# Ewenwan/ORB_SLAM2_SSD_Semantic

Measured on AMD Instinct MI355X. Metric: ORB extract+match frames/sec on 640x480 TUM RGB-D; bit-exact kp/desc, higher is better.
Workload: dtype u8

## Files before the change

orb_slam2_ssd_semantic_amd/csrc/orbfe_api.hip:

```cpp
#include <stdarg.h>
#include <stdlib.h>

#include <algorithm>

#include "orbfe_extractor.h"

static thread_local char t_err[512] = "";

void orbfe_set_error(const char *fmt, ...)
{
    va_list ap;
    va_start(ap, fmt);
    vsnprintf(t_err, sizeof(t_err), fmt, ap);
    va_end(ap);
}

extern "C" const char *orbfe_last_error(void) { return t_err; }
extern "C" int32_t orbfe_version(void) { return ORBFE_VERSION; }

extern "C" const char *orbfe_strerror(orbfe_status s)
{
    switch (s) {
    case ORBFE_OK: return "ok";
    case ORBFE_ERR_ARG: return "invalid argument";
// ... 99 lines not shown
    *flags = 0;
    if (!h->d_misc.p) return ORBFE_OK;
    ORBFE_HIP(wait_last_call(h));
    ORBFE_HIP(hipMemcpy(flags, h->d_misc.p, sizeof(int32_t), hipMemcpyDeviceToHost));
    if (*flags) ORBFE_HIP(hipMemset(h->d_misc.p, 0, sizeof(int32_t)));
    return ORBFE_OK;
}

static orbfe_status create_impl(const orbfe_params *p, hipStream_t borrowed, hipStream_t borrowed_side, bool borrow, orbfe_handle **out);
extern "C" orbfe_status orbfe_create(const orbfe_params *p, orbfe_handle **out) { return create_impl(p, nullptr, nullptr, false, out); }
orbfe_status orbfe_internal_create_on_stream(const orbfe_params *p, void *st, void *side, orbfe_handle **out)
{
    return create_impl(p, (hipStream_t)st, (hipStream_t)side, true, out);
}

static orbfe_status create_impl(const orbfe_params *p, hipStream_t borrowed, hipStream_t borrowed_side, bool borrow, orbfe_handle **out)
{
    if (!p || !out) { orbfe_set_error("null argument"); return ORBFE_ERR_ARG; }
    *out = nullptr;
    OrbPlanIn pin;
    float sigma2[ORBFE_MAX_LEVELS] = {0}, inv_sigma2[ORBFE_MAX_LEVELS] = {0};
    const orbfe_status cs = orb_ctor_tables(p, &pin, sigma2, inv_sigma2);
    if (cs != ORBFE_OK) return cs;
    int dev = p->device;
    const orbfe_status rs = orb_resolve_device(&dev);
    if (rs != ORBFE_OK) return rs;

    orbfe_handle *h = new (std::nothrow) orbfe_handle();
    if (!h) return ORBFE_ERR_NOMEM;
    h->prm = *p;
    h->device = dev;
    DeviceGuard g(dev);
    h->pin = pin;
    memcpy(h->sigma2, sigma2, sizeof(sigma2));
    memcpy(h->inv_sigma2, inv_sigma2, sizeof(inv_sigma2));

    auto fail = [&](orbfe_status s) {
        orbfe_destroy(h);
        return s;
    };
    if (borrow) {
        h->stream = borrowed;
        h->own_stream = false;
        if (borrowed_side) {
            h->side = borrowed_side;
            h->own_side = false;
        }
    }
    for (int r = 0; r < ORBFE_PROF_RING; ++r)
        for (int i = 0; i < ORBFE_EV_N; ++i) h->ev[r][i] = nullptr;
    h->ev_ok = true;
    bool made = true;
    for (const OwnedStream &s : handle_streams(h))
        if (s.own) made = made && hipStreamCreateWithFlags(s.s, hipStreamNonBlocking) == hipSuccess;
    for (int r = 0; r < ORBFE_PROF_RING; ++r)
        for (int i = 0; i < ORBFE_EV_N; ++i) made = made && hipEventCreate(&h->ev[r][i]) == hipSuccess;
    for (hipEvent_t *e : handle_events(h)) made = made && hipEventCreateWithFlags(e, hipEventDisableTiming) == hipSuccess;
    if (!made || h->h_auto.ensure(64) != hipSuccess) {
        orbfe_set_error("stream / event creation failed: %s", hipGetErrorString(hipGetLastError()));
        return fail(ORBFE_ERR_HIP);
    }
#ifdef ORBFE_DEVELOPER
// ... 334 lines not shown
    auto finish = [&]() -> orbfe_status {
        if (ev) {
            ORBFE_HIP(hipEventRecord(ev[5], st));
            h->prof_calls++;
        }
        ORBFE_HIP(hipEventRecord(h->ev_last, st));
        h->last_stream = st;
        h->last_stream_valid = true;
        h->last_gray = d_gray;
        h->last_gray_fstride = (int64_t)frame_stride;
        h->last_gray_pitch = stride;
        h->last_nframes = nframes;
        return ORBFE_OK;
    };
    int ov = h->overlap >= 0 ? h->overlap : (nframes >= 128 ? 2 : 0);
#ifdef ORBFE_DEVELOPER
    if (h->pin.fuse_blur_pyr) {
        ORBFE_HIP(orbk_launch_blur_pyr(a, st));
        if (ev) {
            ORBFE_HIP(hipEventRecord(ev[1], st));
            ORBFE_HIP(hipEventRecord(ev[6], st));
            ORBFE_HIP(hipEventRecord(ev[7], st));
        }
        ORBFE_HIP(orbk_launch_fast(a, st));
        if (ev) ORBFE_HIP(hipEventRecord(ev[2], st));
        ORBFE_HIP(orbk_launch_octree(a, st));
        if (ev) {
            ORBFE_HIP(hipEventRecord(ev[3], st));
            ORBFE_HIP(hipEventRecord(ev[4], st));
        }
        ORBFE_HIP(orbk_launch_describe(a, st));
        return finish();
    }
    const bool ffp = h->fuse_fast_pyr == 1 || h->fuse_fast_pyr == 2;
    const bool fside = h->fuse_fast_pyr == 3;
    if (fside) {
        ORBFE_HIP(orbk_launch_fast_levels(a, 0, 0, 1, st));
        ORBFE_HIP(hipEventRecord(h->ev_fork2, st));
        ORBFE_HIP(hipStreamWaitEvent(h->side, h->ev_fork2, 0));
        ORBFE_HIP(orbk_launch_fast_levels(a, 0, 1, 0, h->side));
        ORBFE_HIP(hipEventRecord(h->ev_join2, h->side));
    }
    if ((ffp || fside) && ov == 1) ov = 2;
#else
    const bool ffp = false, fside = false;
    (void)fside;
#endif
    if (!ffp) ORBFE_HIP(orbk_launch_pyramid(a, st));
    if (ev) ORBFE_HIP(hipEventRecord(ev[1], st));
    auto fork_blur = [&]() -> hipError_t {
// ... 259 lines not shown
```

orb_slam2_ssd_semantic_amd/csrc/orbfe_kernels.h:

```cpp
#pragma once
#include "orbfe_common.h"

struct OrbOpts {
    int32_t pw_rows;
    int32_t pyr_fuse;
    int32_t qt[3];
};

struct OrbLaunch {
    OrbOpts opts;
    const OrbPlan *h_plan;
    const OrbPlan *d_plan;
    const OrbTab *d_tabs;
    const OrbLane *d_flanes;
    const OrbLane *d_flanes_c;
    const OrbLane *d_blanes;
    const OrbLaneR *d_blanesR;
    int32_t nframes;
    const uint8_t *d_gray;
    int64_t gray_fstride;
    int32_t gray_pitch;
    uint8_t *d_pyr;
    uint8_t *d_blur;
    int64_t pyr_fstride;
// ... 38 lines not shown
#endif

struct OrbPyrView {
    int32_t nlevels, device;
    const uint8_t *ptr[ORBFE_MAX_LEVELS];
    int32_t pitch[ORBFE_MAX_LEVELS], w[ORBFE_MAX_LEVELS], h[ORBFE_MAX_LEVELS];
    float scale[ORBFE_MAX_LEVELS], inv_scale[ORBFE_MAX_LEVELS];
    int64_t fstride[ORBFE_MAX_LEVELS];
    int32_t nframes;
};
hipError_t orbk_launch_pad_pyramid(const OrbPyrView &v, const uint32_t *off, uint8_t *d_out, hipStream_t st);
struct orbfe_handle;
int32_t orbfe_internal_pyramid_view(orbfe_handle *h, int frame, OrbPyrView *v);
int32_t orbfe_internal_order_after_last_call(orbfe_handle *h, void *stream);
orbfe_status orbfe_internal_create_on_stream(const orbfe_params *p, void *st, void *side, orbfe_handle **out);
```

orb_slam2_ssd_semantic_amd/csrc/orbfe_pipeline.hip:

```cpp
#include <new>
#include <vector>

#include "orbfe_common.h"
#include "orbfe_kernels.h"
#include "orbfe_matcher.h"

#ifndef ORBFE_PIPE_SIDE_STREAMS
#define ORBFE_PIPE_SIDE_STREAMS 1
#endif

struct orbfe_pipeline {
    orbfe_params prm;
    int device = 0;
    int P = 1;
    int F = 1;
    int cap = 0;
    std::vector<orbfe_handle *> ext;
    std::vector<orbfe_matcher *> mat;
    std::vector<hipStream_t> st;
    std::vector<hipStream_t> side;
    std::vector<hipEvent_t> ev_end;
    std::vector<hipEvent_t> ev_ext;
    std::vector<hipEvent_t> ev_match;
    std::vector<char> ev_match_valid;
    std::vector<char> ev_ext_valid;
    struct Slice { const char *k = nullptr, *d = nullptr, *n = nullptr; size_t kb = 0, db = 0, nb = 0; };
    std::vector<Slice> ev_slice;
    hipEvent_t ev_fork = nullptr;
    int32_t *d_seq = nullptr;
    int seq_len = 0;
    orbfe_keypoint *d_ckps[2] = {nullptr, nullptr};
    uint8_t *d_cdesc[2] = {nullptr, nullptr};
    int32_t *d_cn[2] = {nullptr, nullptr};
    hipEvent_t ev_carry[2] = {nullptr, nullptr};
    hipEvent_t ev_m0[2] = {nullptr, nullptr};
// ... 1 lines not shown
    bool carry_written[2] = {false, false};
    int carry_cur = 0;
    bool have_carry = false;
    const void *carry_src[3] = {nullptr, nullptr, nullptr};
    size_t carry_src_bytes[3] = {0, 0, 0};
    bool joined = true;
    int rot = 0;
    int host_pipes = 1;
    static const int NSETS = 3;
    uint8_t *d_in[NSETS] = {nullptr, nullptr, nullptr};
    orbfe_keypoint *d_okps[NSETS] = {nullptr, nullptr, nullptr};
    uint8_t *d_odesc[NSETS] = {nullptr, nullptr, nullptr};
    int32_t *d_on[NSETS] = {nullptr, nullptr, nullptr}, *d_om[NSETS] = {nullptr, nullptr, nullptr}, *d_onm[NSETS] = {nullptr, nullptr, nullptr};
    size_t in_bytes = 0;
    int out_frames = 0;
    hipStream_t s_in = nullptr, s_out = nullptr;
    hipEvent_t ev_out[NSETS] = {nullptr, nullptr, nullptr};
};

static orbfe_status ensure_events(orbfe_pipeline *pl, int nsub)
{
    while ((int)pl->ev_ext.size() < nsub) {
        hipEvent_t a = nullptr, b = nullptr;
        ORBFE_HIP(hipEventCreateWithFlags(&a, hipEventDisableTiming));
        pl->ev_ext.push_back(a);
        ORBFE_HIP(hipEventCreateWithFlags(&b, hipEventDisableTiming));
        pl->ev_match.push_back(b);
        pl->ev_match_valid.push_back(0);
        pl->ev_ext_valid.push_back(0);
        pl->ev_slice.push_back(orbfe_pipeline::Slice());
    }
    return ORBFE_OK;
}

static orbfe_status ensure_seq(orbfe_pipeline *pl, int nframes)
{
    if (nframes + 1 <= pl->seq_len) return ORBFE_OK;
    for (hipStream_t s : pl->st) ORBFE_HIP(hipStreamSynchronize(s));
    if (pl->d_seq) ORBFE_HIP(hipFree(pl->d_seq));
    pl->d_seq = nullptr;
    pl->seq_len = 0;
    const int len = std::max(nframes + 1, 4096);
    std::vector<int32_t> h((size_t)len);
    for (int i = 0; i < len; ++i) h[(size_t)i] = i - 1;
    ORBFE_HIP(hipMalloc((void **)&pl->d_seq, (size_t)len * sizeof(int32_t)));
    ORBFE_HIP(hipMemcpy(pl->d_seq, h.data(), (size_t)len * sizeof(int32_t), hipMemcpyHostToDevice));
    pl->seq_len = len;
    return ORBFE_OK;
}

extern "C" void orbfe_pipeline_destroy(orbfe_pipeline *pl)
{
    if (!pl) return;
    DeviceGuard g(pl->device);
    for (hipStream_t s : pl->st)
        if (s) (void)hipStreamSynchronize(s);
    for (orbfe_handle *h : pl->ext) orbfe_destroy(h);
    for (orbfe_matcher *m : pl->mat) orbfe_matcher_destroy(m);
    for (hipEvent_t e : pl->ev_end)
        if (e) (void)hipEventDestroy(e);
    for (hipEvent_t e : pl->ev_ext)
        if (e) (void)hipEventDestroy(e);
    for (hipEvent_t e : pl->ev_match)
        if (e) (void)hipEventDestroy(e);
    if (pl->ev_fork) (void)hipEventDestroy(pl->ev_fork);
    for (int k = 0; k < 2; ++k) {
        if (pl->ev_carry[k]) (void)hipEventDestroy(pl->ev_carry[k]);
        if (pl->ev_m0[k]) (void)hipEventDestroy(pl->ev_m0[k]);
        if (pl->d_ckps[k]) (void)hipFree(pl->d_ckps[k]);
        if (pl->d_cdesc[k]) (void)hipFree(pl->d_cdesc[k]);
        if (pl->d_cn[k]) (void)hipFree(pl->d_cn[k]);
    }
    if (pl->d_seq) (void)hipFree(pl->d_seq);
    if (pl->s_in) (void)hipStreamSynchronize(pl->s_in);
    if (pl->s_out) (void)hipStreamSynchronize(pl->s_out);
    for (int k = 0; k < orbfe_pipeline::NSETS; ++k) {
        void *bufs[] = {pl->d_in[k], pl->d_okps[k], pl->d_odesc[k], pl->d_on[k], pl->d_om[k], pl->d_onm[k]};
        for (void *b : bufs)
            if (b) (void)hipFree(b);
        if (pl->ev_out[k]) (void)hipEventDestroy(pl->ev_out[k]);
    }
    if (pl->s_in) (void)hipStreamDestroy(pl->s_in);
    if (pl->s_out) (void)hipStreamDestroy(pl->s_out);
    for (hipStream_t s : pl->st)
        if (s) (void)hipStreamDestroy(s);
    for (hipStream_t s : pl->side)
        if (s) (void)hipStreamDestroy(s);
    delete pl;
}

extern "C" orbfe_status orbfe_pipeline_create(const orbfe_params *p, int32_t npipes, orbfe_pipeline **out)
{
    if (!p || !out || npipes < 1 || npipes > 64) {
        orbfe_set_error("bad argument to orbfe_pipeline_create (1..64 pipes)");
        return ORBFE_ERR_ARG;
    }
    *out = nullptr;
    orbfe_pipeline *pl = new (std::nothrow) orbfe_pipeline();
    if (!pl) return ORBFE_ERR_NOMEM;
    pl->prm = *p;
    pl->P = npipes;
    pl->F = p->max_batch;
    auto fail = [&](orbfe_status s) {
        orbfe_pipeline_destroy(pl);
        return s;
    };
    {
        int dev = p->device;
        const orbfe_status rs = orb_resolve_device(&dev);
        if (rs != ORBFE_OK) return fail(rs);
        pl->device = dev;
        pl->prm.device = dev;
    }
    DeviceGuard g(pl->device);
    for (int i = 0; i < npipes; ++i) {
        hipStream_t st = nullptr;
        hipEvent_t e = nullptr;
        if (hipStreamCreateWithFlags(&st, hipStreamNonBlocking) != hipSuccess) { orbfe_set_error("pipeline stream creation failed"); return fail(ORBFE_ERR_HIP); }
        pl->st.push_back(st);
        if (hipEventCreateWithFlags(&e, hipEventDisableTiming) != hipSuccess) { orbfe_set_error("pipeline event creation failed"); return fail(ORBFE_ERR_HIP); }
        pl->ev_end.push_back(e);
    }
    for (int i = 0; i < std::min(npipes, ORBFE_PIPE_SIDE_STREAMS); ++i) {
        hipStream_t st = nullptr;
        if (hipStreamCreateWithFlags(&st, hipStreamNonBlocking) != hipSuccess) { orbfe_set_error("pipeline stream creation failed"); return fail(ORBFE_ERR_HIP); }
        pl->side.push_back(st);
    }
    for (int i = 0; i < npipes; ++i) {
        orbfe_handle *h = nullptr;
        orbfe_status s = orbfe_internal_create_on_stream(&pl->prm, (void *)pl->st[(size_t)i], (void *)pl->side[(size_t)i % pl->side.size()], &h);
        if (s != ORBFE_OK) return fail(s);
        pl->ext.push_back(h);
        orbfe_matcher *m = nullptr;
        s = orbfe_internal_matcher_create_on_stream(pl->device, (void *)pl->st[(size_t)i], &m);
        if (s != ORBFE_OK) return fail(s);
        pl->mat.push_back(m);
    }
    {
        int32_t feat[ORBFE_MAX_LEVELS];
        int worst = 0;
        if (orbfe_get_features_per_level(pl->ext[0], feat) == ORBFE_OK)
            for (int l = 0; l < pl->prm.nlevels; ++l) worst += std::max(feat[l] + 2, 4 * ORBFE_MAX_ROOTS);
        pl->cap = std::max(orbfe_keypoint_capacity(pl->ext[0]), (worst + 63) & ~63);
    }
    if (hipEventCreateWithFlags(&pl->ev_fork, hipEventDisableTiming) != hipSuccess) { orbfe_set_error("pipeline event creation failed"); return fail(ORBFE_ERR_HIP); }
    for (int k = 0; k < 2; ++k) {
        if (hipEventCreateWithFlags(&pl->ev_carry[k], hipEventDisableTiming) != hipSuccess ||
            hipEventCreateWithFlags(&pl->ev_m0[k], hipEventDisableTiming) != hipSuccess ||
            hipMalloc((void **)&pl->d_ckps[k], (size_t)pl->cap * sizeof(orbfe_keypoint)) != hipSuccess ||
            hipMalloc((void **)&pl->d_cdesc[k], (size_t)pl->cap * 32) != hipSuccess ||
            hipMalloc((void **)&pl->d_cn[k], 64) != hipSuccess) {
            orbfe_set_error("pipeline carry buffers: %s", hipGetErrorString(hipGetLastError()));
            return fail(ORBFE_ERR_NOMEM);
        }
        (void)hipMemset(pl->d_cn[k], 0, 64);
    }
    orbfe_status s = ensure_seq(pl, 4095);
    if (s != ORBFE_OK) return fail(s);
    *out = pl;
    return ORBFE_OK;
}

extern "C" int32_t orbfe_pipeline_pipes(const orbfe_pipeline *pl) { return pl ? pl->P : 0; }
extern "C" int32_t orbfe_pipeline_capacity(const orbfe_pipeline *pl) { return pl ? pl->cap : 0; }
extern "C" int32_t orbfe_pipeline_sub_batch(const orbfe_pipeline *pl) { return pl ? pl->F : 0; }
extern "C" orbfe_handle *orbfe_pipeline_extractor(orbfe_pipeline *pl, int32_t pipe)
{
    return (pl && pipe >= 0 && pipe < pl->P) ? pl->ext[(size_t)pipe] : nullptr;
}
extern "C" orbfe_matcher *orbfe_pipeline_matcher(orbfe_pipeline *pl, int32_t pipe)
{
    return (pl && pipe >= 0 && pipe < pl->P) ? pl->mat[(size_t)pipe] : nullptr;
}

extern "C" orbfe_status orbfe_pipeline_set_host_pipes(orbfe_pipeline *pl, int32_t n)
{
    if (!pl || n < 1) return ORBFE_ERR_ARG;
    pl->host_pipes = std::min(n, pl->P);
    return ORBFE_OK;
}

extern "C" orbfe_status orbfe_pipeline_reset_sequence(orbfe_pipeline *pl)
{
    if (!pl) return ORBFE_ERR_ARG;
    pl->have_carry = false;
    return ORBFE_OK;
}

extern "C" orbfe_status orbfe_pipeline_join(orbfe_pipeline *pl, void *stream)
{
    if (!pl) return ORBFE_ERR_ARG;
    DeviceGuard g(pl->device);
    for (int p = 0; p < pl->P; ++p) ORBFE_HIP(hipStreamWaitEvent((hipStream_t)stream, pl->ev_end[(size_t)p], 0));
    pl->joined = true;
    return ORBFE_OK;
}

extern "C" orbfe_status orbfe_pipeline_synchronize(orbfe_pipeline *pl)
{
    if (!pl) return ORBFE_ERR_ARG;
    DeviceGuard g(pl->device);
    for (hipStream_t s : pl->st) ORBFE_HIP(hipStreamSynchronize(s));
    return ORBFE_OK;
}

extern "C" orbfe_status orbfe_pipeline_get_overflow(orbfe_pipeline *pl, int32_t *flags)
{
    if (!pl || !flags) return ORBFE_ERR_ARG;
    *flags = 0;
    for (orbfe_handle *h : pl->ext) {
        int32_t f = 0;
        const orbfe_status s = orbfe_get_overflow(h, &f);
        if (s != ORBFE_OK) return s;
        *flags |= f;
    }
    return ORBFE_OK;
}

extern "C" orbfe_status orbfe_pipeline_extract_match_device(orbfe_pipeline *pl, const uint8_t *d_gray, int32_t nframes, int32_t w,
                                                            int32_t ht, int32_t stride, size_t frame_stride, orbfe_keypoint *d_kps,
                                                            uint8_t *d_desc, int32_t cap, int32_t *d_n_out, int32_t *d_match,
                                                            int32_t *d_nmatches, float nnratio, int32_t th, int32_t check_ori,
                                                            int32_t flags, void *stream)
{
    if (!pl || !d_gray || !d_kps || !d_desc || !d_n_out || nframes < 1 || cap < 1 || (d_match && !d_nmatches)) {
        orbfe_set_error("bad argument to orbfe_pipeline_extract_match_device");
        return ORBFE_ERR_ARG;
    }
    DeviceGuard g(pl->device);
    const int F = pl->F, P = pl->P;
    const int nsub = (nframes + F - 1) / F;
    orbfe_status s = ensure_events(pl, nsub + 1);
    if (s != ORBFE_OK) return s;
    s = ensure_seq(pl, nframes);
    if (s != ORBFE_OK) return s;
    hipStream_t cs = (hipStream_t)stream;
    const bool match = d_match != nullptr;
    const bool cont = (flags & ORBFE_PIPE_CONTINUE) != 0 && pl->have_carry && match;
    const int rd = pl->carry_cur, wr = pl->carry_cur ^ 1;

    ORBFE_HIP(hipEventRecord(pl->ev_fork, cs));
    for (int p = 0; p < P; ++p) ORBFE_HIP(hipStreamWaitEvent(pl->st[(size_t)p], pl->ev_fork, 0));
    auto bail = [&](orbfe_status e) {
        for (hipStream_t x : pl->st) (void)hipStreamSynchronize(x);
        pl->have_carry = false;
        pl->m0_valid[0] = pl->m0_valid[1] = false;
        pl->joined = true;
        return e;
    };
    auto overlaps = [](const void *a, size_t na, const void *b, size_t nb) {
        const char *pa = (const char *)a, *pb = (const char *)b;
        return a && b && pa < pb + nb && pb < pa + na;
    };

    for (int j = 0; j < nsub; ++j) {
        const int p = (pl->rot + j) % P;
        hipStream_t st = pl->st[(size_t)p];
        const int lo = j * F, nf = std::min(F, nframes - lo);
        {
            const char *ok = (const char *)(d_kps + (size_t)lo * cap), *od = (const char *)(d_desc + (size_t)lo * cap * 32), *on = (const char *)(d_n_out + lo);
            const size_t okb = (size_t)nf * cap * sizeof(orbfe_keypoint), odb = (size_t)nf * cap * 32, onb = (size_t)nf * sizeof(int32_t);
            auto wait_index = [&](size_t i) -> hipError_t {
                hipError_t e = hipSuccess;
                if (pl->ev_ext_valid[i]) e = hipStreamWaitEvent(st, pl->ev_ext[i], 0);
                if (e == hipSuccess && pl->ev_match_valid[i]) e = hipStreamWaitEvent(st, pl->ev_match[i], 0);
                if (e == hipSuccess && i + 1 < pl->ev_match_valid.size() && pl->ev_match_valid[i + 1]) e = hipStreamWaitEvent(st, pl->ev_match[i + 1], 0);
                return e;
            };
            ORBFE_HIP(wait_index((size_t)j));
            for (size_t i = 0; i < pl->ev_slice.size(); ++i) {
                const orbfe_pipeline::Slice &si = pl->ev_slice[i];
                if ((int)i != j && si.k && (overlaps(si.k, si.kb, ok, okb) || overlaps(si.d, si.db, od, odb) || overlaps(si.n, si.nb, on, onb)))
// ... 33 lines not shown
                                                 pl->d_seq + 1, pl->d_seq + 1, 1, nnratio, th, check_ori, d_match, d_nmatches, (void *)st);
                if (s != ORBFE_OK) return bail(s);
                ORBFE_HIP(hipEventRecord(pl->ev_m0[rd], st));
                pl->m0_valid[rd] = true;
            } else {
                ORBFE_HIP(hipMemsetAsync(d_match, 0xFF, (size_t)cap * sizeof(int32_t), st));
                ORBFE_HIP(hipMemsetAsync(d_nmatches, 0, sizeof(int32_t), st));
            }
        }
        ORBFE_HIP(hipEventRecord(pl->ev_match[(size_t)j], st));
        pl->ev_match_valid[(size_t)j] = 1;
    }

    {
        const int jl = nsub - 1;
        hipStream_t st = pl->st[(size_t)((pl->rot + jl) % P)];
        const size_t last = (size_t)nframes - 1;
        if (pl->m0_valid[wr]) {
            ORBFE_HIP(hipStreamWaitEvent(st, pl->ev_m0[wr], 0));
            pl->m0_valid[wr] = false;
        }
        if (pl->carry_written[wr]) ORBFE_HIP(hipStreamWaitEvent(st, pl->ev_carry[wr], 0));
        ORBFE_HIP(hipMemcpyAsync(pl->d_ckps[wr], d_kps + last * cap, (size_t)std::min(cap, pl->cap) * sizeof(orbfe_keypoint),
                                 hipMemcpyDeviceToDevice, st));
        ORBFE_HIP(hipMemcpyAsync(pl->d_cdesc[wr], d_desc + last * cap * 32, (size_t)std::min(cap, pl->cap) * 32, hipMemcpyDeviceToDevice, st));
        ORBFE_HIP(hipMemcpyAsync(pl->d_cn[wr], d_n_out + last, sizeof(int32_t), hipMemcpyDeviceToDevice, st));
        ORBFE_HIP(hipEventRecord(pl->ev_carry[wr], st));
        pl->carry_written[wr] = true;
        pl->carry_cur = wr;
        pl->have_carry = true;
        pl->carry_src[0] = d_kps + last * cap;
        pl->carry_src_bytes[0] = (size_t)std::min(cap, pl->cap) * sizeof(orbfe_keypoint);
        pl->carry_src[1] = d_desc + last * cap * 32;
        pl->carry_src_bytes[1] = (size_t)std::min(cap, pl->cap) * 32;
        pl->carry_src[2] = d_n_out + last;
        pl->carry_src_bytes[2] = sizeof(int32_t);
    }
    for (int p = 0; p < P; ++p) ORBFE_HIP(hipEventRecord(pl->ev_end[(size_t)p], pl->st[(size_t)p]));
    pl->joined = false;
    pl->rot = (pl->rot + nsub) % P;
    if (!(flags & ORBFE_PIPE_NO_JOIN)) return orbfe_pipeline_join(pl, stream);
    return ORBFE_OK;
}

static orbfe_status ensure_host_sets(orbfe_pipeline *pl, int w, int ht)
{
    const size_t need = (size_t)pl->F * w * ht;
    if (need <= pl->in_bytes && pl->out_frames == pl->F) return ORBFE_OK;
    if (!pl->s_in) ORBFE_HIP(hipStreamCreateWithFlags(&pl->s_in, hipStreamNonBlocking));
    if (!pl->s_out) ORBFE_HIP(hipStreamCreateWithFlags(&pl->s_out, hipStreamNonBlocking));
    ORBFE_HIP(hipStreamSynchronize(pl->s_in));
    ORBFE_HIP(hipStreamSynchronize(pl->s_out));
    for (hipStream_t st : pl->st) ORBFE_HIP(hipStreamSynchronize(st));
    const size_t F = (size_t)pl->F, cap = (size_t)pl->cap;
    for (int k = 0; k < orbfe_pipeline::NSETS; ++k) {
        if (pl->d_in[k]) ORBFE_HIP(hipFree(pl->d_in[k]));
        pl->d_in[k] = nullptr;
        ORBFE_HIP(hipMalloc((void **)&pl->d_in[k], need + 64));
        if (!pl->ev_out[k]) ORBFE_HIP(hipEventCreateWithFlags(&pl->ev_out[k], hipEventDisableTiming));
        if (!pl->d_okps[k]) {
            ORBFE_HIP(hipMalloc((void **)&pl->d_okps[k], F * cap * sizeof(orbfe_keypoint)));
            ORBFE_HIP(hipMalloc((void **)&pl->d_odesc[k], F * cap * 32));
            ORBFE_HIP(hipMalloc((void **)&pl->d_on[k], F * sizeof(int32_t)));
            ORBFE_HIP(hipMalloc((void **)&pl->d_om[k], F * cap * sizeof(int32_t)));
            ORBFE_HIP(hipMalloc((void **)&pl->d_onm[k], F * sizeof(int32_t)));
        }
    }
    pl->in_bytes = need;
// ... 3 lines not shown

extern "C" orbfe_status orbfe_pipeline_extract_match(orbfe_pipeline *pl, const uint8_t *const *grays, int32_t nframes, int32_t w, int32_t ht,
                                                     int32_t stride, orbfe_keypoint *kps, uint8_t *desc, int32_t cap, int32_t *n_out,
                                                     int32_t *match, int32_t *nmatches, float nnratio, int32_t th, int32_t check_ori,
                                                     int32_t flags)
{
    if (!pl || !grays || !kps || !desc || !n_out || nframes < 1 || w < 1 || ht < 1 || stride < w || (match && !nmatches)) {
        orbfe_set_error("bad argument to orbfe_pipeline_extract_match");
        return ORBFE_ERR_ARG;
    }
    if (cap < pl->cap) {
        orbfe_set_error("orbfe_pipeline_extract_match: cap %d below orbfe_pipeline_capacity() = %d", cap, pl->cap);
        return ORBFE_ERR_CAP;
    }
    DeviceGuard g(pl->device);
    orbfe_status s = ensure_host_sets(pl, w, ht);
    if (s != ORBFE_OK) return s;
    const int F = pl->F, pc = pl->cap;
    const size_t fbytes = (size_t)w * ht;
    const int nchunks = (nframes + F - 1) / F;
    struct Drain {
        orbfe_pipeline *pl;
        ~Drain()
        {
            if (pl->s_in) (void)hipStreamSynchronize(pl->s_in);
            for (hipStream_t st : pl->st) (void)hipStreamSynchronize(st);
            if (pl->s_out) (void)hipStreamSynchronize(pl->s_out);
        }
    } drain{pl};
    for (int c = 0; c < nchunks; ++c) {
        const int k = c % orbfe_pipeline::NSETS, lo = c * F, nf = std::min(F, nframes - lo);
        if (c >= orbfe_pipeline::NSETS) ORBFE_HIP(hipStreamWaitEvent(pl->s_in, pl->ev_out[k], 0));
        bool contiguous = stride == w;
        for (int f = 1; f < nf && contiguous; ++f) contiguous = grays[lo + f] == grays[lo + f - 1] + fbytes;
        if (contiguous) {
            ORBFE_HIP(hipMemcpyAsync(pl->d_in[k], grays[lo], fbytes * nf, hipMemcpyHostToDevice, pl->s_in));
        } else {
            for (int f = 0; f < nf; ++f)
                ORBFE_HIP(hipMemcpy2DAsync(pl->d_in[k] + fbytes * f, (size_t)w, grays[lo + f], (size_t)stride, (size_t)w, (size_t)ht,
                                           hipMemcpyHostToDevice, pl->s_in));
        }
        const int fl = ((c > 0 || (flags & ORBFE_PIPE_CONTINUE)) ? ORBFE_PIPE_CONTINUE : 0) | ORBFE_PIPE_NO_JOIN;
        pl->rot = c % std::max(1, std::min(pl->host_pipes, pl->P));
        s = orbfe_pipeline_extract_match_device(pl, pl->d_in[k], nf, w, ht, w, fbytes, pl->d_okps[k], pl->d_odesc[k], pc, pl->d_on[k],
                                                match ? pl->d_om[k] : nullptr, match ? pl->d_onm[k] : nullptr, nnratio, th, check_ori, fl,
                                                (void *)pl->s_in);
        if (s != ORBFE_OK) return s;
        s = orbfe_pipeline_join(pl, (void *)pl->s_out);
        if (s != ORBFE_OK) return s;
        ORBFE_HIP(hipMemcpyAsync(n_out + lo, pl->d_on[k], (size_t)nf * sizeof(int32_t), hipMemcpyDeviceToHost, pl->s_out));
        auto rows_out = [&](void *dst, const void *src, size_t elem) -> hipError_t {
            if (cap == pc) return hipMemcpyAsync(dst, src, (size_t)nf * pc * elem, hipMemcpyDeviceToHost, pl->s_out);
            return hipMemcpy2DAsync(dst, (size_t)cap * elem, src, (size_t)pc * elem, (size_t)pc * elem, (size_t)nf, hipMemcpyDeviceToHost, pl->s_out);
        };
        ORBFE_HIP(rows_out(kps + (size_t)lo * cap, pl->d_okps[k], sizeof(orbfe_keypoint)));
        ORBFE_HIP(rows_out(desc + (size_t)lo * cap * 32, pl->d_odesc[k], 32));
        if (match) {
            ORBFE_HIP(rows_out(match + (size_t)lo * cap, pl->d_om[k], sizeof(int32_t)));
            ORBFE_HIP(hipMemcpyAsync(nmatches + lo, pl->d_onm[k], (size_t)nf * sizeof(int32_t), hipMemcpyDeviceToHost, pl->s_out));
        }
        ORBFE_HIP(hipEventRecord(pl->ev_out[k], pl->s_out));
    }
    ORBFE_HIP(hipStreamSynchronize(pl->s_out));
    int32_t ovf = 0;
    s = orbfe_pipeline_get_overflow(pl, &ovf);
    if (s != ORBFE_OK) return s;
    if (ovf) {
        orbfe_set_error("device-side capacity overflow %d in orbfe_pipeline_extract_match", ovf);
        return ORBFE_ERR_CAP;
    }
    return ORBFE_OK;
}
```

orb_slam2_ssd_semantic_amd/pipeline.py:

```python
import ctypes as C

from . import _ffi
from ._ffi import Handle, OrbfeParams, check
from .extractor import ORBextractor
from .matcher import ORBmatcher


class FramePipeline(Handle):
    _HANDLE, _DESTROY = "_p", "orbfe_pipeline_destroy"
    CONTINUE, NO_JOIN = _ffi.PIPE_CONTINUE, _ffi.PIPE_NO_JOIN

    def __init__(self, nfeatures=1000, scaleFactor=1.2, nlevels=8, iniThFAST=20, minThFAST=7, *, max_width=640, max_height=480,
                 sub_batch=1024, npipes=3, device=-1, blur_rounding=0, nnratio=0.9, th=100, check_ori=True):
        self._L = _ffi.lib()
        self._p = C.c_void_p()
        prm = OrbfeParams(nfeatures, scaleFactor, nlevels, iniThFAST, minThFAST, max_width, max_height, sub_batch, device,
                          blur_rounding)
        check(self._L.orbfe_pipeline_create(C.byref(prm), npipes, C.byref(self._p)), "orbfe_pipeline_create")
        self.npipes, self.sub_batch, self.blur_rounding = npipes, sub_batch, blur_rounding
        self.cap = int(self._L.orbfe_pipeline_capacity(self._p))
        self.nnratio, self.th, self.check_ori = float(nnratio), int(th), bool(check_ori)
        kw = dict(max_width=max_width, max_height=max_height, max_batch=sub_batch, device=device, blur_rounding=blur_rounding)
        self.extractors = [ORBextractor(nfeatures, scaleFactor, nlevels, iniThFAST, minThFAST,
                                        _borrow=self._L.orbfe_pipeline_extractor(self._p, i), **kw) for i in range(npipes)]
        self.matchers = [ORBmatcher(nnratio, check_ori, _borrow=self._L.orbfe_pipeline_matcher(self._p, i)) for i in range(npipes)]

    def close(self):
        if getattr(self, "_p", None):
            for o in self.extractors + self.matchers:
                o.close()
        super().close()

    @property
# ... 5 lines not shown

    def extract_match_device(self, d_gray, nframes, w, h, stride, frame_stride, d_kps, d_desc, cap, d_n, d_match=None, d_nmatches=None,
                             flags=0, stream=None):
        check(self._L.orbfe_pipeline_extract_match_device(self._p, d_gray, nframes, w, h, stride, frame_stride, d_kps, d_desc, cap, d_n,
                                                          d_match, d_nmatches, self.nnratio, self.th, int(self.check_ori), flags,
                                                          stream), "orbfe_pipeline_extract_match_device")

    def extract_match(self, frame_ptrs, nframes, w, h, stride, kps_ptr, desc_ptr, cap, n_ptr, match_ptr=None, nmatches_ptr=None, flags=0):
        check(self._L.orbfe_pipeline_extract_match(self._p, frame_ptrs, nframes, w, h, stride, kps_ptr, desc_ptr, cap, n_ptr, match_ptr,
                                                   nmatches_ptr, self.nnratio, self.th, int(self.check_ori), flags),
              "orbfe_pipeline_extract_match")

    def set_host_pipes(self, n):
        check(self._L.orbfe_pipeline_set_host_pipes(self._p, int(n)), "orbfe_pipeline_set_host_pipes")

    def join(self, stream=None):
        check(self._L.orbfe_pipeline_join(self._p, stream), "orbfe_pipeline_join")

    def synchronize(self):
        check(self._L.orbfe_pipeline_synchronize(self._p), "orbfe_pipeline_synchronize")

    def reset_sequence(self):
        check(self._L.orbfe_pipeline_reset_sequence(self._p), "orbfe_pipeline_reset_sequence")

    def overflow(self):
        f = C.c_int32(0)
        check(self._L.orbfe_pipeline_get_overflow(self._p, C.byref(f)), "orbfe_pipeline_get_overflow")
        return f.value

    def set_fast_mode(self, mode, collect_stats=False):
# ... 7 lines not shown
```

Baseline: 307,100.

## Plan pipeline streams to fit the hardware queue count and reuse spare streams

```diff
diff --git a/orb_slam2_ssd_semantic_amd/csrc/orbfe_api.hip b/orb_slam2_ssd_semantic_amd/csrc/orbfe_api.hip
--- a/orb_slam2_ssd_semantic_amd/csrc/orbfe_api.hip
+++ b/orb_slam2_ssd_semantic_amd/csrc/orbfe_api.hip
@@ -137,6 +137,13 @@
     return create_impl(p, (hipStream_t)st, (hipStream_t)side, true, out);
 }
 
+orbfe_status orbfe_internal_set_side_stream(orbfe_handle *h, void *side)
+{
+    if (!h || h->own_side) return ORBFE_ERR_ARG;
+    h->side = (hipStream_t)side;
+    return ORBFE_OK;
+}
+
 static orbfe_status create_impl(const orbfe_params *p, hipStream_t borrowed, hipStream_t borrowed_side, bool borrow, orbfe_handle **out)
 {
     if (!p || !out) { orbfe_set_error("null argument"); return ORBFE_ERR_ARG; }
@@ -165,10 +172,8 @@
     if (borrow) {
         h->stream = borrowed;
         h->own_stream = false;
-        if (borrowed_side) {
-            h->side = borrowed_side;
-            h->own_side = false;
-        }
+        h->side = borrowed_side;
+        h->own_side = false;
     }
     for (int r = 0; r < ORBFE_PROF_RING; ++r)
         for (int i = 0; i < ORBFE_EV_N; ++i) h->ev[r][i] = nullptr;
@@ -533,6 +538,7 @@
         return ORBFE_OK;
     };
     int ov = h->overlap >= 0 ? h->overlap : (nframes >= 128 ? 2 : 0);
+    if (!h->side) ov = 0;
 #ifdef ORBFE_DEVELOPER
     if (h->pin.fuse_blur_pyr) {
         ORBFE_HIP(orbk_launch_blur_pyr(a, st));
@@ -552,7 +558,7 @@
         return finish();
     }
     const bool ffp = h->fuse_fast_pyr == 1 || h->fuse_fast_pyr == 2;
-    const bool fside = h->fuse_fast_pyr == 3;
+    const bool fside = h->fuse_fast_pyr == 3 && h->side;
     if (fside) {
         ORBFE_HIP(orbk_launch_fast_levels(a, 0, 0, 1, st));
         ORBFE_HIP(hipEventRecord(h->ev_fork2, st));
diff --git a/orb_slam2_ssd_semantic_amd/csrc/orbfe_kernels.h b/orb_slam2_ssd_semantic_amd/csrc/orbfe_kernels.h
--- a/orb_slam2_ssd_semantic_amd/csrc/orbfe_kernels.h
+++ b/orb_slam2_ssd_semantic_amd/csrc/orbfe_kernels.h
@@ -76,3 +76,4 @@
 int32_t orbfe_internal_pyramid_view(orbfe_handle *h, int frame, OrbPyrView *v);
 int32_t orbfe_internal_order_after_last_call(orbfe_handle *h, void *stream);
 orbfe_status orbfe_internal_create_on_stream(const orbfe_params *p, void *st, void *side, orbfe_handle **out);
+orbfe_status orbfe_internal_set_side_stream(orbfe_handle *h, void *side);
diff --git a/orb_slam2_ssd_semantic_amd/csrc/orbfe_pipe_plan.h b/orb_slam2_ssd_semantic_amd/csrc/orbfe_pipe_plan.h
--- /dev/null
+++ b/orb_slam2_ssd_semantic_amd/csrc/orbfe_pipe_plan.h
@@ -0,0 +1,58 @@
+#pragma once
+
+#include <errno.h>
+#include <stdint.h>
+#include <stdlib.h>
+
+#define ORBFE_PIPE_MAX_PIPES 64
+#define ORBFE_PIPE_DEFAULT_QUEUES 4
+#define ORBFE_PIPE_MAX_QUEUES 32
+#define ORBFE_PIPE_COPY_STREAMS 2
+
+struct OrbPipePlan {
+    int32_t P, Q, copies;
+    int32_t S;
+    int32_t P_eff;
+    int32_t side;
+    int32_t first, side_index , nstreams;
+    int32_t stream_of_pipe[ORBFE_PIPE_MAX_PIPES];
+};
+
+static inline int32_t orb_pipe_parse_queues(const char *text)
+{
+    if (!text || !*text) return ORBFE_PIPE_DEFAULT_QUEUES;
+    char *end = nullptr;
+    errno = 0;
+    const long long v = strtoll(text, &end, 10);
+    if (end == text) return ORBFE_PIPE_DEFAULT_QUEUES;
+    while (*end == ' ' || *end == '\t' || *end == '\n' || *end == '\r') ++end;
+    if (*end) return ORBFE_PIPE_DEFAULT_QUEUES;
+    if (errno == ERANGE) return v > 0 ? ORBFE_PIPE_MAX_QUEUES : ORBFE_PIPE_DEFAULT_QUEUES;
+    if (v < 1) return ORBFE_PIPE_DEFAULT_QUEUES;
+    return v > ORBFE_PIPE_MAX_QUEUES ? ORBFE_PIPE_MAX_QUEUES : (int32_t)v;
+}
+
+static inline int32_t orb_pipe_env_queues()
+{
+    static const int32_t q = orb_pipe_parse_queues(getenv("GPU_MAX_HW_QUEUES"));
+    return q;
+}
+
+static inline bool orb_pipe_plan(int32_t P, int32_t Q, bool copies, OrbPipePlan *out)
+{
+    if (!out || P < 1 || P > ORBFE_PIPE_MAX_PIPES) return false;
+    OrbPipePlan pl;
+    pl.P = P;
+    pl.Q = Q < 1 ? 1 : (Q > ORBFE_PIPE_MAX_QUEUES ? ORBFE_PIPE_MAX_QUEUES : Q);
+    pl.copies = copies ? 1 : 0;
+    pl.first = copies ? ORBFE_PIPE_COPY_STREAMS : 0;
+    const int32_t left = pl.Q - pl.first < 1 ? 1 : pl.Q - pl.first;
+    pl.side = left >= 2 ? 1 : 0;
+    pl.S = left >= P + 1 ? P : (pl.side ? left - 1 : 1);
+    pl.P_eff = P < pl.S ? P : pl.S;
+    pl.side_index = pl.side ? pl.first + pl.S : -1;
+    pl.nstreams = pl.first + pl.S + pl.side;
+    for (int32_t i = 0; i < ORBFE_PIPE_MAX_PIPES; ++i) pl.stream_of_pipe[i] = i < P ? i % pl.S : -1;
+    *out = pl;
+    return true;
+}
diff --git a/orb_slam2_ssd_semantic_amd/csrc/orbfe_pipeline.hip b/orb_slam2_ssd_semantic_amd/csrc/orbfe_pipeline.hip
--- a/orb_slam2_ssd_semantic_amd/csrc/orbfe_pipeline.hip
+++ b/orb_slam2_ssd_semantic_amd/csrc/orbfe_pipeline.hip
@@ -1,24 +1,43 @@
+#include <mutex>
 #include <new>
+#include <utility>
 #include <vector>
 
 #include "orbfe_common.h"
 #include "orbfe_kernels.h"
 #include "orbfe_matcher.h"
-
-#ifndef ORBFE_PIPE_SIDE_STREAMS
-#define ORBFE_PIPE_SIDE_STREAMS 1
-#endif
+#include "orbfe_pipe_plan.h"
+
+static std::mutex g_spare_mu;
+static std::vector<std::pair<int, hipStream_t>> g_spare;
+
+static hipStream_t take_spare_stream(int device)
+{
+    std::lock_guard<std::mutex> lk(g_spare_mu);
+    for (size_t i = g_spare.size(); i-- > 0;)
+        if (g_spare[i].first == device) {
+            hipStream_t s = g_spare[i].second;
+            g_spare.erase(g_spare.begin() + (ptrdiff_t)i);
+            return s;
+        }
+    return nullptr;
+}
 
 struct orbfe_pipeline {
     orbfe_params prm;
     int device = 0;
     int P = 1;
+    int Q = ORBFE_PIPE_DEFAULT_QUEUES;
+    OrbPipePlan cur;
+    bool cur_valid = false;
     int F = 1;
     int cap = 0;
     std::vector<orbfe_handle *> ext;
     std::vector<orbfe_matcher *> mat;
-    std::vector<hipStream_t> st;
-    std::vector<hipStream_t> side;
+    std::vector<hipStream_t> pool;
+    hipStream_t stream_of(int pipe) const { return pool[(size_t)(cur.first + cur.stream_of_pipe[pipe])]; }
+    hipStream_t side() const { return cur.side ? pool[(size_t)cur.side_index] : nullptr; }
+    std::vector<char> ev_end_valid;
     std::vector<hipEvent_t> ev_end;
     std::vector<hipEvent_t> ev_ext;
     std::vector<hipEvent_t> ev_match;
@@ -50,7 +69,8 @@
     int32_t *d_on[NSETS] = {nullptr, nullptr, nullptr}, *d_om[NSETS] = {nullptr, nullptr, nullptr}, *d_onm[NSETS] = {nullptr, nullptr, nullptr};
     size_t in_bytes = 0;
     int out_frames = 0;
-    hipStream_t s_in = nullptr, s_out = nullptr;
+    hipStream_t s_in() const { return pool[0]; }
+    hipStream_t s_out() const { return pool[1]; }
     hipEvent_t ev_out[NSETS] = {nullptr, nullptr, nullptr};
 };
 
@@ -72,7 +92,7 @@
 static orbfe_status ensure_seq(orbfe_pipeline *pl, int nframes)
 {
     if (nframes + 1 <= pl->seq_len) return ORBFE_OK;
-    for (hipStream_t s : pl->st) ORBFE_HIP(hipStreamSynchronize(s));
+    for (hipStream_t s : pl->pool) ORBFE_HIP(hipStreamSynchronize(s));
     if (pl->d_seq) ORBFE_HIP(hipFree(pl->d_seq));
     pl->d_seq = nullptr;
     pl->seq_len = 0;
@@ -89,7 +109,7 @@
 {
     if (!pl) return;
     DeviceGuard g(pl->device);
-    for (hipStream_t s : pl->st)
+    for (hipStream_t s : pl->pool)
         if (s) (void)hipStreamSynchronize(s);
     for (orbfe_handle *h : pl->ext) orbfe_destroy(h);
     for (orbfe_matcher *m : pl->mat) orbfe_matcher_destroy(m);
@@ -108,26 +128,44 @@
         if (pl->d_cn[k]) (void)hipFree(pl->d_cn[k]);
     }
     if (pl->d_seq) (void)hipFree(pl->d_seq);
-    if (pl->s_in) (void)hipStreamSynchronize(pl->s_in);
-    if (pl->s_out) (void)hipStreamSynchronize(pl->s_out);
     for (int k = 0; k < orbfe_pipeline::NSETS; ++k) {
         void *bufs[] = {pl->d_in[k], pl->d_okps[k], pl->d_odesc[k], pl->d_on[k], pl->d_om[k], pl->d_onm[k]};
         for (void *b : bufs)
             if (b) (void)hipFree(b);
         if (pl->ev_out[k]) (void)hipEventDestroy(pl->ev_out[k]);
     }
-    if (pl->s_in) (void)hipStreamDestroy(pl->s_in);
-    if (pl->s_out) (void)hipStreamDestroy(pl->s_out);
-    for (hipStream_t s : pl->st)
-        if (s) (void)hipStreamDestroy(s);
-    for (hipStream_t s : pl->side)
-        if (s) (void)hipStreamDestroy(s);
+    {
+        std::lock_guard<std::mutex> lk(g_spare_mu);
+        for (size_t i = pl->pool.size(); i-- > 0;)
+            if (pl->pool[i]) g_spare.push_back(std::make_pair(pl->device, pl->pool[i]));
+    }
     delete pl;
 }
 
-extern "C" orbfe_status orbfe_pipeline_create(const orbfe_params *p, int32_t npipes, orbfe_pipeline **out)
-{
-    if (!p || !out || npipes < 1 || npipes > 64) {
+static orbfe_status apply_plan(orbfe_pipeline *pl, const OrbPipePlan &plan)
+{
+    const bool same = pl->cur_valid && pl->cur.copies == plan.copies && pl->cur.S == plan.S && pl->cur.side == plan.side &&
+                      pl->cur.P_eff == plan.P_eff;
+    if (same) return ORBFE_OK;
+    for (hipStream_t s : pl->pool) ORBFE_HIP(hipStreamSynchronize(s));
+    while ((int)pl->pool.size() < plan.nstreams) {
+        hipStream_t st = take_spare_stream(pl->device);
+        if (!st && hipStreamCreateWithFlags(&st, hipStreamNonBlocking) != hipSuccess) { orbfe_set_error("pipeline stream creation failed"); return ORBFE_ERR_HIP; }
+        pl->pool.push_back(st);
+    }
+    pl->cur = plan;
+    pl->cur_valid = true;
+    pl->rot %= plan.P_eff;
+    for (int i = 0; i < pl->P && i < (int)pl->ext.size(); ++i) {
+        const orbfe_status s = orbfe_internal_set_side_stream(pl->ext[(size_t)i], (void *)pl->side());
+        if (s != ORBFE_OK) return s;
+    }
+    return ORBFE_OK;
+}
+
+extern "C" orbfe_status orbfe_internal_pipeline_create_queues(const orbfe_params *p, int32_t npipes, int32_t queues, orbfe_pipeline **out)
+{
+    if (!p || !out || npipes < 1 || npipes > ORBFE_PIPE_MAX_PIPES) {
         orbfe_set_error("bad argument to orbfe_pipeline_create (1..64 pipes)");
         return ORBFE_ERR_ARG;
     }
@@ -136,6 +174,7 @@
     if (!pl) return ORBFE_ERR_NOMEM;
     pl->prm = *p;
     pl->P = npipes;
+    pl->Q = std::min(std::max(queues, 1), ORBFE_PIPE_MAX_QUEUES);
     pl->F = p->max_batch;
     auto fail = [&](orbfe_status s) {
         orbfe_pipeline_destroy(pl);
@@ -149,26 +188,25 @@
         pl->prm.device = dev;
     }
     DeviceGuard g(pl->device);
+    {
+        OrbPipePlan plan;
+        if (!orb_pipe_plan(npipes, pl->Q, false, &plan)) return fail(ORBFE_ERR_ARG);
+        const orbfe_status s = apply_plan(pl, plan);
+        if (s != ORBFE_OK) return fail(s);
+    }
     for (int i = 0; i < npipes; ++i) {
-        hipStream_t st = nullptr;
         hipEvent_t e = nullptr;
-        if (hipStreamCreateWithFlags(&st, hipStreamNonBlocking) != hipSuccess) { orbfe_set_error("pipeline stream creation failed"); return fail(ORBFE_ERR_HIP); }
-        pl->st.push_back(st);
         if (hipEventCreateWithFlags(&e, hipEventDisableTiming) != hipSuccess) { orbfe_set_error("pipeline event creation failed"); return fail(ORBFE_ERR_HIP); }
         pl->ev_end.push_back(e);
-    }
-    for (int i = 0; i < std::min(npipes, ORBFE_PIPE_SIDE_STREAMS); ++i) {
-        hipStream_t st = nullptr;
-        if (hipStreamCreateWithFlags(&st, hipStreamNonBlocking) != hipSuccess) { orbfe_set_error("pipeline stream creation failed"); return fail(ORBFE_ERR_HIP); }
-        pl->side.push_back(st);
+        pl->ev_end_valid.push_back(0);
     }
     for (int i = 0; i < npipes; ++i) {
         orbfe_handle *h = nullptr;
-        orbfe_status s = orbfe_internal_create_on_stream(&pl->prm, (void *)pl->st[(size_t)i], (void *)pl->side[(size_t)i % pl->side.size()], &h);
+        orbfe_status s = orbfe_internal_create_on_stream(&pl->prm, (void *)pl->stream_of(i), (void *)pl->side(), &h);
         if (s != ORBFE_OK) return fail(s);
         pl->ext.push_back(h);
         orbfe_matcher *m = nullptr;
-        s = orbfe_internal_matcher_create_on_stream(pl->device, (void *)pl->st[(size_t)i], &m);
+        s = orbfe_internal_matcher_create_on_stream(pl->device, (void *)pl->stream_of(i), &m);
         if (s != ORBFE_OK) return fail(s);
         pl->mat.push_back(m);
     }
@@ -197,6 +235,31 @@
     return ORBFE_OK;
 }
 
+extern "C" orbfe_status orbfe_pipeline_create(const orbfe_params *p, int32_t npipes, orbfe_pipeline **out)
+{
+    return orbfe_internal_pipeline_create_queues(p, npipes, orb_pipe_env_queues(), out);
+}
+
+extern "C" int32_t orbfe_internal_pipe_plan(int32_t npipes, int32_t queues, int32_t copies, int32_t *out)
+{
+    OrbPipePlan plan;
+    if (!out || !orb_pipe_plan(npipes, queues, copies != 0, &plan)) return ORBFE_ERR_ARG;
+    const int32_t head[9] = {plan.P, plan.Q, plan.copies, plan.S, plan.P_eff, plan.side, plan.first, plan.side_index, plan.nstreams};
+    for (int i = 0; i < 9; ++i) out[i] = head[i];
+    for (int i = 0; i < ORBFE_PIPE_MAX_PIPES; ++i) out[9 + i] = plan.stream_of_pipe[i];
+    return ORBFE_OK;
+}
+extern "C" int32_t orbfe_internal_pipe_parse_queues(const char *text) { return orb_pipe_parse_queues(text); }
+extern "C" int32_t orbfe_internal_pipe_env_queues(void) { return orb_pipe_env_queues(); }
+extern "C" orbfe_status orbfe_internal_pipeline_streams(const orbfe_pipeline *pl, int32_t *streams, int32_t *eff_pipes, int32_t *side)
+{
+    if (!pl || !pl->cur_valid) return ORBFE_ERR_ARG;
+    if (streams) *streams = pl->cur.S;
+    if (eff_pipes) *eff_pipes = pl->cur.P_eff;
+    if (side) *side = pl->cur.side;
+    return ORBFE_OK;
+}
+
 extern "C" int32_t orbfe_pipeline_pipes(const orbfe_pipeline *pl) { return pl ? pl->P : 0; }
 extern "C" int32_t orbfe_pipeline_capacity(const orbfe_pipeline *pl) { return pl ? pl->cap : 0; }
 extern "C" int32_t orbfe_pipeline_sub_batch(const orbfe_pipeline *pl) { return pl ? pl->F : 0; }
@@ -227,7 +290,8 @@
 {
     if (!pl) return ORBFE_ERR_ARG;
     DeviceGuard g(pl->device);
-    for (int p = 0; p < pl->P; ++p) ORBFE_HIP(hipStreamWaitEvent((hipStream_t)stream, pl->ev_end[(size_t)p], 0));
+    for (int p = 0; p < pl->P; ++p)
+        if (pl->ev_end_valid[(size_t)p]) ORBFE_HIP(hipStreamWaitEvent((hipStream_t)stream, pl->ev_end[(size_t)p], 0));
     pl->joined = true;
     return ORBFE_OK;
 }
@@ -236,7 +300,7 @@
 {
     if (!pl) return ORBFE_ERR_ARG;
     DeviceGuard g(pl->device);
-    for (hipStream_t s : pl->st) ORBFE_HIP(hipStreamSynchronize(s));
+    for (hipStream_t s : pl->pool) ORBFE_HIP(hipStreamSynchronize(s));
     return ORBFE_OK;
 }
 
@@ -253,18 +317,11 @@
     return ORBFE_OK;
 }
 
-extern "C" orbfe_status orbfe_pipeline_extract_match_device(orbfe_pipeline *pl, const uint8_t *d_gray, int32_t nframes, int32_t w,
-                                                            int32_t ht, int32_t stride, size_t frame_stride, orbfe_keypoint *d_kps,
-                                                            uint8_t *d_desc, int32_t cap, int32_t *d_n_out, int32_t *d_match,
-                                                            int32_t *d_nmatches, float nnratio, int32_t th, int32_t check_ori,
-                                                            int32_t flags, void *stream)
-{
-    if (!pl || !d_gray || !d_kps || !d_desc || !d_n_out || nframes < 1 || cap < 1 || (d_match && !d_nmatches)) {
-        orbfe_set_error("bad argument to orbfe_pipeline_extract_match_device");
-        return ORBFE_ERR_ARG;
-    }
-    DeviceGuard g(pl->device);
-    const int F = pl->F, P = pl->P;
+static orbfe_status run_device(orbfe_pipeline *pl, const uint8_t *d_gray, int32_t nframes, int32_t w, int32_t ht, int32_t stride,
+                               size_t frame_stride, orbfe_keypoint *d_kps, uint8_t *d_desc, int32_t cap, int32_t *d_n_out, int32_t *d_match,
+                               int32_t *d_nmatches, float nnratio, int32_t th, int32_t check_ori, int32_t flags, void *stream)
+{
+    const int F = pl->F, P = pl->cur.P_eff;
     const int nsub = (nframes + F - 1) / F;
     orbfe_status s = ensure_events(pl, nsub + 1);
     if (s != ORBFE_OK) return s;
@@ -276,9 +333,9 @@
     const int rd = pl->carry_cur, wr = pl->carry_cur ^ 1;
 
     ORBFE_HIP(hipEventRecord(pl->ev_fork, cs));
-    for (int p = 0; p < P; ++p) ORBFE_HIP(hipStreamWaitEvent(pl->st[(size_t)p], pl->ev_fork, 0));
+    for (int p = 0; p < P; ++p) ORBFE_HIP(hipStreamWaitEvent(pl->stream_of(p), pl->ev_fork, 0));
     auto bail = [&](orbfe_status e) {
-        for (hipStream_t x : pl->st) (void)hipStreamSynchronize(x);
+        for (hipStream_t x : pl->pool) (void)hipStreamSynchronize(x);
         pl->have_carry = false;
         pl->m0_valid[0] = pl->m0_valid[1] = false;
         pl->joined = true;
@@ -291,7 +348,7 @@
 
     for (int j = 0; j < nsub; ++j) {
         const int p = (pl->rot + j) % P;
-        hipStream_t st = pl->st[(size_t)p];
+        hipStream_t st = pl->stream_of(p);
         const int lo = j * F, nf = std::min(F, nframes - lo);
         {
             const char *ok = (const char *)(d_kps + (size_t)lo * cap), *od = (const char *)(d_desc + (size_t)lo * cap * 32), *on = (const char *)(d_n_out + lo);
@@ -355,7 +412,7 @@
 
     {
         const int jl = nsub - 1;
-        hipStream_t st = pl->st[(size_t)((pl->rot + jl) % P)];
+        hipStream_t st = pl->stream_of((pl->rot + jl) % P);
         const size_t last = (size_t)nframes - 1;
         if (pl->m0_valid[wr]) {
             ORBFE_HIP(hipStreamWaitEvent(st, pl->ev_m0[wr], 0));
@@ -377,22 +434,40 @@
         pl->carry_src[2] = d_n_out + last;
         pl->carry_src_bytes[2] = sizeof(int32_t);
     }
-    for (int p = 0; p < P; ++p) ORBFE_HIP(hipEventRecord(pl->ev_end[(size_t)p], pl->st[(size_t)p]));
+    for (int p = 0; p < P; ++p) {
+        ORBFE_HIP(hipEventRecord(pl->ev_end[(size_t)p], pl->stream_of(p)));
+        pl->ev_end_valid[(size_t)p] = 1;
+    }
     pl->joined = false;
     pl->rot = (pl->rot + nsub) % P;
     if (!(flags & ORBFE_PIPE_NO_JOIN)) return orbfe_pipeline_join(pl, stream);
     return ORBFE_OK;
 }
 
+extern "C" orbfe_status orbfe_pipeline_extract_match_device(orbfe_pipeline *pl, const uint8_t *d_gray, int32_t nframes, int32_t w,
+                                                            int32_t ht, int32_t stride, size_t frame_stride, orbfe_keypoint *d_kps,
+                                                            uint8_t *d_desc, int32_t cap, int32_t *d_n_out, int32_t *d_match,
+                                                            int32_t *d_nmatches, float nnratio, int32_t th, int32_t check_ori,
+                                                            int32_t flags, void *stream)
+{
+    if (!pl || !d_gray || !d_kps || !d_desc || !d_n_out || nframes < 1 || cap < 1 || (d_match && !d_nmatches)) {
+        orbfe_set_error("bad argument to orbfe_pipeline_extract_match_device");
+        return ORBFE_ERR_ARG;
+    }
+    DeviceGuard g(pl->device);
+    OrbPipePlan plan;
+    if (!orb_pipe_plan(pl->P, pl->Q, false, &plan)) return ORBFE_ERR_ARG;
+    const orbfe_status s = apply_plan(pl, plan);
+    if (s != ORBFE_OK) return s;
+    return run_device(pl, d_gray, nframes, w, ht, stride, frame_stride, d_kps, d_desc, cap, d_n_out, d_match, d_nmatches, nnratio, th, check_ori,
+                      flags, stream);
+}
+
 static orbfe_status ensure_host_sets(orbfe_pipeline *pl, int w, int ht)
 {
     const size_t need = (size_t)pl->F * w * ht;
     if (need <= pl->in_bytes && pl->out_frames == pl->F) return ORBFE_OK;
-    if (!pl->s_in) ORBFE_HIP(hipStreamCreateWithFlags(&pl->s_in, hipStreamNonBlocking));
-    if (!pl->s_out) ORBFE_HIP(hipStreamCreateWithFlags(&pl->s_out, hipStreamNonBlocking));
-    ORBFE_HIP(hipStreamSynchronize(pl->s_in));
-    ORBFE_HIP(hipStreamSynchronize(pl->s_out));
-    for (hipStream_t st : pl->st) ORBFE_HIP(hipStreamSynchronize(st));
+    for (hipStream_t st : pl->pool) ORBFE_HIP(hipStreamSynchronize(st));
     const size_t F = (size_t)pl->F, cap = (size_t)pl->cap;
     for (int k = 0; k < orbfe_pipeline::NSETS; ++k) {
         if (pl->d_in[k]) ORBFE_HIP(hipFree(pl->d_in[k]));
@@ -426,7 +501,11 @@
         return ORBFE_ERR_CAP;
     }
     DeviceGuard g(pl->device);
-    orbfe_status s = ensure_host_sets(pl, w, ht);
+    OrbPipePlan plan;
+    if (!orb_pipe_plan(std::max(1, std::min(pl->host_pipes, pl->P)), pl->Q, true, &plan)) return ORBFE_ERR_ARG;
+    orbfe_status s = apply_plan(pl, plan);
+    if (s != ORBFE_OK) return s;
+    s = ensure_host_sets(pl, w, ht);
     if (s != ORBFE_OK) return s;
     const int F = pl->F, pc = pl->cap;
     const size_t fbytes = (size_t)w * ht;
@@ -435,45 +514,42 @@
         orbfe_pipeline *pl;
         ~Drain()
         {
-            if (pl->s_in) (void)hipStreamSynchronize(pl->s_in);
-            for (hipStream_t st : pl->st) (void)hipStreamSynchronize(st);
-            if (pl->s_out) (void)hipStreamSynchronize(pl->s_out);
+            for (hipStream_t st : pl->pool) (void)hipStreamSynchronize(st);
         }
     } drain{pl};
     for (int c = 0; c < nchunks; ++c) {
         const int k = c % orbfe_pipeline::NSETS, lo = c * F, nf = std::min(F, nframes - lo);
-        if (c >= orbfe_pipeline::NSETS) ORBFE_HIP(hipStreamWaitEvent(pl->s_in, pl->ev_out[k], 0));
+        if (c >= orbfe_pipeline::NSETS) ORBFE_HIP(hipStreamWaitEvent(pl->s_in(), pl->ev_out[k], 0));
         bool contiguous = stride == w;
         for (int f = 1; f < nf && contiguous; ++f) contiguous = grays[lo + f] == grays[lo + f - 1] + fbytes;
         if (contiguous) {
-            ORBFE_HIP(hipMemcpyAsync(pl->d_in[k], grays[lo], fbytes * nf, hipMemcpyHostToDevice, pl->s_in));
+            ORBFE_HIP(hipMemcpyAsync(pl->d_in[k], grays[lo], fbytes * nf, hipMemcpyHostToDevice, pl->s_in()));
         } else {
             for (int f = 0; f < nf; ++f)
                 ORBFE_HIP(hipMemcpy2DAsync(pl->d_in[k] + fbytes * f, (size_t)w, grays[lo + f], (size_t)stride, (size_t)w, (size_t)ht,
-                                           hipMemcpyHostToDevice, pl->s_in));
+                                           hipMemcpyHostToDevice, pl->s_in()));
         }
         const int fl = ((c > 0 || (flags & ORBFE_PIPE_CONTINUE)) ? ORBFE_PIPE_CONTINUE : 0) | ORBFE_PIPE_NO_JOIN;
-        pl->rot = c % std::max(1, std::min(pl->host_pipes, pl->P));
-        s = orbfe_pipeline_extract_match_device(pl, pl->d_in[k], nf, w, ht, w, fbytes, pl->d_okps[k], pl->d_odesc[k], pc, pl->d_on[k],
-                                                match ? pl->d_om[k] : nullptr, match ? pl->d_onm[k] : nullptr, nnratio, th, check_ori, fl,
-                                                (void *)pl->s_in);
+        pl->rot = c % pl->cur.P_eff;
+        s = run_device(pl, pl->d_in[k], nf, w, ht, w, fbytes, pl->d_okps[k], pl->d_odesc[k], pc, pl->d_on[k], match ? pl->d_om[k] : nullptr,
+                       match ? pl->d_onm[k] : nullptr, nnratio, th, check_ori, fl, (void *)pl->s_in());
         if (s != ORBFE_OK) return s;
-        s = orbfe_pipeline_join(pl, (void *)pl->s_out);
+        s = orbfe_pipeline_join(pl, (void *)pl->s_out());
         if (s != ORBFE_OK) return s;
-        ORBFE_HIP(hipMemcpyAsync(n_out + lo, pl->d_on[k], (size_t)nf * sizeof(int32_t), hipMemcpyDeviceToHost, pl->s_out));
+        ORBFE_HIP(hipMemcpyAsync(n_out + lo, pl->d_on[k], (size_t)nf * sizeof(int32_t), hipMemcpyDeviceToHost, pl->s_out()));
         auto rows_out = [&](void *dst, const void *src, size_t elem) -> hipError_t {
-            if (cap == pc) return hipMemcpyAsync(dst, src, (size_t)nf * pc * elem, hipMemcpyDeviceToHost, pl->s_out);
-            return hipMemcpy2DAsync(dst, (size_t)cap * elem, src, (size_t)pc * elem, (size_t)pc * elem, (size_t)nf, hipMemcpyDeviceToHost, pl->s_out);
+            if (cap == pc) return hipMemcpyAsync(dst, src, (size_t)nf * pc * elem, hipMemcpyDeviceToHost, pl->s_out());
+            return hipMemcpy2DAsync(dst, (size_t)cap * elem, src, (size_t)pc * elem, (size_t)pc * elem, (size_t)nf, hipMemcpyDeviceToHost, pl->s_out());
         };
         ORBFE_HIP(rows_out(kps + (size_t)lo * cap, pl->d_okps[k], sizeof(orbfe_keypoint)));
         ORBFE_HIP(rows_out(desc + (size_t)lo * cap * 32, pl->d_odesc[k], 32));
         if (match) {
             ORBFE_HIP(rows_out(match + (size_t)lo * cap, pl->d_om[k], sizeof(int32_t)));
-            ORBFE_HIP(hipMemcpyAsync(nmatches + lo, pl->d_onm[k], (size_t)nf * sizeof(int32_t), hipMemcpyDeviceToHost, pl->s_out));
-        }
-        ORBFE_HIP(hipEventRecord(pl->ev_out[k], pl->s_out));
-    }
-    ORBFE_HIP(hipStreamSynchronize(pl->s_out));
+            ORBFE_HIP(hipMemcpyAsync(nmatches + lo, pl->d_onm[k], (size_t)nf * sizeof(int32_t), hipMemcpyDeviceToHost, pl->s_out()));
+        }
+        ORBFE_HIP(hipEventRecord(pl->ev_out[k], pl->s_out()));
+    }
+    ORBFE_HIP(hipStreamSynchronize(pl->s_out()));
     int32_t ovf = 0;
     s = orbfe_pipeline_get_overflow(pl, &ovf);
     if (s != ORBFE_OK) return s;
diff --git a/orb_slam2_ssd_semantic_amd/pipeline.py b/orb_slam2_ssd_semantic_amd/pipeline.py
--- a/orb_slam2_ssd_semantic_amd/pipeline.py
+++ b/orb_slam2_ssd_semantic_amd/pipeline.py
@@ -11,12 +11,17 @@
     CONTINUE, NO_JOIN = _ffi.PIPE_CONTINUE, _ffi.PIPE_NO_JOIN
 
     def __init__(self, nfeatures=1000, scaleFactor=1.2, nlevels=8, iniThFAST=20, minThFAST=7, *, max_width=640, max_height=480,
-                 sub_batch=1024, npipes=3, device=-1, blur_rounding=0, nnratio=0.9, th=100, check_ori=True):
+                 sub_batch=1024, npipes=3, device=-1, blur_rounding=0, nnratio=0.9, th=100, check_ori=True, _queues=None):
         self._L = _ffi.lib()
         self._p = C.c_void_p()
         prm = OrbfeParams(nfeatures, scaleFactor, nlevels, iniThFAST, minThFAST, max_width, max_height, sub_batch, device,
                           blur_rounding)
-        check(self._L.orbfe_pipeline_create(C.byref(prm), npipes, C.byref(self._p)), "orbfe_pipeline_create")
+        if _queues is None:
+            check(self._L.orbfe_pipeline_create(C.byref(prm), npipes, C.byref(self._p)), "orbfe_pipeline_create")
+        else:
+            f = self._L.orbfe_internal_pipeline_create_queues
+            f.argtypes = [C.POINTER(OrbfeParams), C.c_int32, C.c_int32, C.POINTER(C.c_void_p)]
+            check(f(C.byref(prm), npipes, int(_queues), C.byref(self._p)), "orbfe_internal_pipeline_create_queues")
         self.npipes, self.sub_batch, self.blur_rounding = npipes, sub_batch, blur_rounding
         self.cap = int(self._L.orbfe_pipeline_capacity(self._p))
         self.nnratio, self.th, self.check_ori = float(nnratio), int(th), bool(check_ori)
@@ -52,6 +57,13 @@
     def set_host_pipes(self, n):
         check(self._L.orbfe_pipeline_set_host_pipes(self._p, int(n)), "orbfe_pipeline_set_host_pipes")
 
+    def streams(self):
+        v = [C.c_int32(0) for _ in range(3)]
+        f = self._L.orbfe_internal_pipeline_streams
+        f.argtypes = [C.c_void_p] + [C.POINTER(C.c_int32)] * 3
+        check(f(self._p, *[C.byref(x) for x in v]), "orbfe_internal_pipeline_streams")
+        return tuple(x.value for x in v)
+
     def join(self, stream=None):
         check(self._L.orbfe_pipeline_join(self._p, stream), "orbfe_pipeline_join")
 
```

Measured after the change: 315,900 (median of 6 runs). +2.9%, better.
